# goalheart/ionic-mpnn

Measured on AMD Instinct MI355X. Metric: molecule-graph pairs/sec (fwd), batch 4096 per MI355X, higher is better.
Workload: dtype f32 (bf16x9 emulation)

## Files before the change

### include/impnn.h

```cpp
#ifndef IMPNN_H_
#define IMPNN_H_

#include <stddef.h>
#include <stdint.h>

#ifdef __cplusplus
extern "C" {
#endif

#define IMPNN_OK 0
#define IMPNN_E_BADARG (-1)
#define IMPNN_E_UNSUPPORTED (-2)
#define IMPNN_E_LAUNCH (-3)
#define IMPNN_E_WORKSPACE (-4)

typedef void* impnn_stream_t;

#define IMPNN_ABI_VERSION 3
int impnn_abi_version(void);
const char* impnn_last_error_string(void);
const char* impnn_target_arch(void);

int impnn_embed_gather(const int32_t* ids, const float* table, float* out, int64_t rows,
                       int32_t vocab, int32_t dim, impnn_stream_t stream);
// ... 97 lines not shown
int impnn_encoder_workspace_bytes(int32_t n_ions, int32_t B, int32_t N, int32_t E, int32_t D,
                                  int32_t K, int32_t S, int32_t Vb, int32_t mode, int32_t workgroups,
                                  size_t* bytes);
int impnn_encoder_fused(int32_t n_ions, const int32_t* const* atom_ids,
                        const int32_t* const* bond_ids, const int32_t* const* conn,
                        const float* atom_table, int32_t Va, const float* bond_table, int32_t Vb,
                        const float* const* weights, int32_t mode, float* const* pooled, int32_t B,
                        int32_t N, int32_t E, int32_t D, int32_t K, int32_t S, float ln_eps,
                        int32_t workgroups, void* workspace, size_t workspace_bytes,
                        impnn_stream_t stream);

size_t impnn_encoder_prepared_bytes(int32_t D, int32_t S, int32_t Vb, int32_t mode);
int impnn_encoder_prepare_weights(const float* weights, const float* bond_table, int32_t D, int32_t K,
                                  int32_t S, int32_t Vb, int32_t mode, void* prepared,
                                  size_t prepared_bytes, impnn_stream_t stream);
int impnn_encoder_fused_prepared(int32_t n_ions, const int32_t* const* atom_ids,
                                 const int32_t* const* bond_ids, const int32_t* const* conn,
                                 const float* atom_table, int32_t Va, const float* bond_table,
                                 int32_t Vb, const void* const* prepared, int32_t mode,
                                 float* const* pooled, int32_t B, int32_t N, int32_t E, int32_t D,
                                 int32_t K, int32_t S, float ln_eps, int32_t workgroups, void* workspace,
                                 size_t workspace_bytes, impnn_stream_t stream);

int64_t impnn_model_head_floats(int32_t kind, int32_t D, int32_t F, int32_t Mx);
int impnn_model_head(int32_t kind, const float* pooled_cat, const float* pooled_an,
                     const float* temperature, const float* head_weights, float* out, int32_t B,
                     int32_t D, int32_t F, int32_t Mx, impnn_stream_t stream);

int impnn_head_ion_mix(int32_t kind, int32_t ion, const float* pooled, const float* head_weights, float* mix,
                       int32_t M, int32_t D, int32_t F, int32_t Mx, impnn_stream_t stream);
// ... 232 lines not shown
```

### ionic_mpnn_amd/_lib.py

```python
from __future__ import annotations

import ctypes as C
import threading
from pathlib import Path

import torch

import os

_LIB_PATH = Path(os.environ.get("IMPNN_LIB") or Path(__file__).resolve().parent / "csrc" / "libimpnn.so")
_lock = threading.Lock()
_lib = None

i32, i64, u64, f32, vp, sz = C.c_int32, C.c_int64, C.c_uint64, C.c_float, C.c_void_p, C.c_size_t
PP = C.POINTER(vp)

_GU_FWD = [vp] * 10 + [f32, vp]
_GU_BWD = [vp] * 9 + [f32] + [vp] * 5 + [i64]
_ROWS = [vp, vp]
_DROP = [f32, u64, vp, i32]

SIGNATURES = {
    "impnn_abi_version": (C.c_int, []),
    "impnn_last_error_string": (C.c_char_p, []),
# ... 5 lines not shown
    "impnn_reduce_scatter_add": (C.c_int, [vp, vp, i32, vp, i32, i32, i32, i32, vp]),
    "impnn_bmm_fused": (C.c_int, [vp, vp, vp, vp, vp, i32, i32, i32, i32, i32, vp]),
    "impnn_gated_update": (C.c_int, _GU_FWD + [i64, i32, vp]),
    "impnn_gated_update_rows": (C.c_int, _GU_FWD + _ROWS + [i64, i32, vp]),
    "impnn_kept_rows": (C.c_int, [vp, vp, vp, vp, i32, i32, i32, i32, vp]),
    "impnn_row_index_fill": (C.c_int, [vp, vp, vp, vp, i32, i32, vp]),
    "impnn_global_sum_pool": (C.c_int, [vp, vp, vp, i32, i32, i32, vp]),
    "impnn_encoder_step_floats": (i64, [i32, i32]),
    "impnn_encoder_plan_overflow_offset": (sz, []),
    "impnn_encoder_workspace_bytes": (C.c_int, [i32] * 10 + [C.POINTER(sz)]),
    "impnn_encoder_fused": (C.c_int, [i32, C.POINTER(vp), C.POINTER(vp), C.POINTER(vp), vp, i32, vp, i32,
                                      C.POINTER(vp), i32, C.POINTER(vp), i32, i32, i32, i32, i32, i32, f32, i32, vp,
                                      sz, vp]),
    "impnn_encoder_prepared_bytes": (sz, [i32, i32, i32, i32]),
    "impnn_encoder_prepare_weights": (C.c_int, [vp, vp, i32, i32, i32, i32, i32, vp, sz, vp]),
    "impnn_encoder_fused_prepared": (C.c_int, [i32, C.POINTER(vp), C.POINTER(vp), C.POINTER(vp), vp, i32, vp, i32,
                                               C.POINTER(vp), i32, C.POINTER(vp), i32, i32, i32, i32, i32, i32, f32,
                                               i32, vp, sz, vp]),
    "impnn_encoder_plan": (C.c_int, [i32, C.POINTER(vp), C.POINTER(vp), C.POINTER(vp), i32, i32, i32, i32, i32, i32,
                                     i32, i32, i32, i32, vp, sz, vp, vp]),
    "impnn_encoder_run": (C.c_int, [i32, C.POINTER(vp), vp, i32, vp, i32, C.POINTER(vp), i32, C.POINTER(vp), i32, i32,
                                    i32, i32, i32, i32, f32, vp, vp, sz, vp]),
    "impnn_model_head_floats": (i64, [i32, i32, i32, i32]),
    "impnn_model_head": (C.c_int, [i32, vp, vp, vp, vp, vp, i32, i32, i32, i32, vp]),
    "impnn_head_ion_mix": (C.c_int, [i32, i32, vp, vp, vp, i32, i32, i32, i32, vp]),
    "impnn_head_grid": (C.c_int, [i32, vp, vp, vp, vp, vp, vp, i32, i32, i32, i32, i32, i32, vp]),
    "impnn_model_head_tensors": (C.c_int, [i32, vp, vp, vp, PP, vp, i32, i32, i32, i32, vp]),
    "impnn_model_head_bwd": (C.c_int, [i32, vp, vp, vp, PP, vp, vp, vp, PP, i32, i32, i32, i32, vp]),
    "impnn_model_head_bwd_max_floats": (i64, []),
    "impnn_model_head_loss_workspace_floats": (i64, [i32]),
# ... 166 lines not shown
```

### ionic_mpnn_amd/csrc/api.hip

```cpp
#include <cstring>
#include <vector>

#include <cstddef>

#include "common.h"
#include "encoder_layout.h"

namespace impnn {

char* error_buffer() {
  static thread_local char buf[512] = {0};
  return buf;
}

int fail(int code, const char* fmt, ...) {
  va_list ap;
  va_start(ap, fmt);
  vsnprintf(error_buffer(), 512, fmt, ap);
  va_end(ap);
  return code;
}

namespace {
struct Profiler {
// ... 421 lines not shown
                                  int32_t Vb, int32_t mode, void* prepared, size_t prepared_bytes,
                                  impnn_stream_t stream) {
  REQUIRE(D > 0 && K > 0 && S >= 0 && Vb > 0, "bad shape");
  REQUIRE(mode >= 0 && mode <= 3, "mode must be 0 (f32), 1 (f16x2), 2 (f32 typed) or 3 (f32x3 typed)");
  if (!encoder_fused_supported(mode, 1, 0, D, K, S, mode >= 2 ? Vb : 1))
    return fail(IMPNN_E_UNSUPPORTED, "encoder_prepare_weights: mode=%d D=%d K=%d Vb=%d not covered", mode, D, K, Vb);
  if (S == 0) return IMPNN_OK;
  REQUIRE(weights && prepared && (mode < 2 || bond_table), "null pointer");
  REQUIRE(aligned16(prepared), "prepared buffer must be 16B aligned");
  if (prepared_bytes < encoder_prepared_bytes(mode, D, S, Vb))
    return fail(IMPNN_E_WORKSPACE, "encoder_prepare_weights: buffer %zu < %zu bytes", prepared_bytes,
                encoder_prepared_bytes(mode, D, S, Vb));
  return launch_encoder_prepare(weights, bond_table, D, K, S, Vb, mode, prepared, as_stream(stream));
}

int impnn_encoder_fused_prepared(int32_t n_ions, const int32_t* const* atom_ids, const int32_t* const* bond_ids,
                                 const int32_t* const* conn, const float* atom_table, int32_t Va,
                                 const float* bond_table, int32_t Vb, const void* const* prepared, int32_t mode,
                                 float* const* pooled, int32_t B, int32_t N, int32_t E, int32_t D, int32_t K,
                                 int32_t S, float ln_eps, int32_t workgroups, void* workspace, size_t workspace_bytes,
                                 impnn_stream_t stream) {
  return encoder_common(__func__, n_ions, atom_ids, bond_ids, conn, atom_table, Va, bond_table, Vb, nullptr, prepared,
                        mode, pooled, B, N, E, D, K, S, ln_eps, workgroups, nullptr, nullptr, workspace,
                        workspace_bytes, stream);
}

int64_t impnn_model_head_floats(int32_t kind, int32_t D, int32_t F, int32_t Mx) {
  if (D <= 0 || F <= 0 || Mx <= 0 || (kind != 0 && kind != 1)) return -1;
  const int64_t common = 2 * ((int64_t)D * F + F) + 2 * ((int64_t)F * Mx + Mx);
  return common + (kind == 0 ? (int64_t)Mx * 3 + 3 : (int64_t)Mx * F + F + F + 1);
// ... 979 lines not shown
```

### ionic_mpnn_amd/csrc/common.h

```cpp
#pragma once

#include <hip/hip_runtime.h>

#include <cstdarg>
#include <cstdint>
#include <cstdio>

#include "../../include/impnn.h"

namespace impnn {

char* error_buffer();
int fail(int code, const char* fmt, ...);

inline hipStream_t as_stream(impnn_stream_t s) { return reinterpret_cast<hipStream_t>(s); }

inline int check_launch(const char* what) {
  hipError_t e = hipGetLastError();
  if (e != hipSuccess) return fail(IMPNN_E_LAUNCH, "%s: %s", what, hipGetErrorString(e));
  return IMPNN_OK;
}

inline bool aligned16(const void* p) { return (reinterpret_cast<uintptr_t>(p) & 15u) == 0; }

// ... 361 lines not shown
  const float* atom_table;
  const float* bond_table;
  int Va, Vb, B, N, E, D, K, S;
  float ln_eps;
  void* workspace;
  size_t workspace_bytes;
};
bool encoder_fused_supported(int mode, int N, int E, int D, int K, int S, int Vb);
int encoder_workgroups(int n_ions, int B, int requested, int N, int E, int mode);
size_t encoder_fused_workspace_bytes(int mode, int n_ions, int B, int N, int E, int D, int S, int Vb, int nwg);
int launch_encoder_fused(const EncoderArgs& a, hipStream_t s);
int launch_encoder_phase(const EncoderArgs& a, hipStream_t s, bool plan_phase);
size_t encoder_prepared_bytes(int mode, int D, int S, int Vb);
int launch_encoder_prepare(const float* weights, const float* bond_table, int D, int K, int S, int Vb, int mode,
                           void* prepared, hipStream_t s);
int ensure_lds_limit(const void* kern, int slot);
int device_compute_units();
inline int gu_wide_tile_rows(int64_t rows) { return rows < 8192 ? 16 : 64; }
bool encoder_wide_supported(int N, int E, int D, int K, int S, int Vb);
size_t encoder_wide_workspace_bytes(int n_ions, int B, int N, int E, int D, int S, int Vb, bool x3);
size_t encoder_wide_prepared_bytes(int D, int S, int Vb, bool x3);
int launch_encoder_wide_prepare(const float* weights, const float* bond_table, int D, int K, int S, int Vb, bool x3,
                                void* prepared, hipStream_t s);
int launch_encoder_wide(const EncoderArgs& a, hipStream_t s);

}
```

### ionic_mpnn_amd/csrc/encoder_fused.hip

```cpp
#include <atomic>
#include <cstdlib>

#include "encoder_device.h"
#include "encoder_layout.h"

namespace impnn {
namespace enc {

namespace {

struct H8 {
  half8 hi, lo;
};
__device__ __forceinline__ H8 split8(const float* v) {
  typedef __fp16 h2_t __attribute__((ext_vector_type(2)));
  union U {
    h2_t h;
    unsigned u;
  };
  union {
    half8 v8;
    unsigned u[4];
  } hi, lo;
#pragma unroll
// ... 396 lines not shown
    stamp[2] = t_steps;
    stamp[3] = t_pool;
    stamp[4] = (unsigned long long)(c_end - c_begin);
    stamp[7] = __builtin_amdgcn_s_memtime();
  }
}

}

}

bool encoder_typed_supported(int N, int E, int D, int S, int Vb);
size_t encoder_typed_prepared_bytes(int S, int Vb, bool x3);
int launch_encoder_typed_prepare(const float* weights, const float* bond_table, int K, int S, int Vb, bool x3,
                                 void* prepared, hipStream_t s);
int launch_encoder_typed_run(const EncoderArgs& a, const enc::Ws& w, hipStream_t s);

bool encoder_fused_supported(int mode, int N, int E, int D, int K, int S, int Vb) {
  using namespace enc;
  if ((mode == 2 || mode == 3) && D != kD) return encoder_wide_supported(N, E, D, K, S, Vb);
  if (mode == 2 || mode == 3) return K >= 1 && encoder_typed_supported(N, E, D, S, Vb);
  if (mode != 0 && mode != 1) return false;
  if (D != kD || K < 1 || K > kKMax || S < 0) return false;
  if (N < 1 || N > 0xffff || E < 0) return false;
  if (Vb < 1 || Vb > 0xffff || (int64_t)Vb * kKMax > kTbCapFloats) return false;
  const int vrmax = vr_max_of(N, E);
  if (vrmax > kRCap / 2) return false;
  return true;
}

// ... 51 lines not shown
  return (size_t)(S > 0 ? S : 1) * enc::kImgSlot * sizeof(float);
}

int launch_encoder_prepare(const float* weights, const float* bond_table, int D, int K, int S, int Vb, int mode,
                           void* prepared, hipStream_t s) {
  if (S <= 0) return IMPNN_OK;
  if (D != enc::kD) return launch_encoder_wide_prepare(weights, bond_table, D, K, S, Vb, mode == 3, prepared, s);
  if (mode >= 2) return launch_encoder_typed_prepare(weights, bond_table, K, S, Vb, mode == 3, prepared, s);
  enc::ImageParams ip{};
  ip.weights = weights;
  ip.img = static_cast<float*>(prepared);
  ip.K = K;
  ip.mode = mode == 1 ? 1 : 0;
  ip.step_floats = impnn_encoder_step_floats(D, K);
  return enc::launch_weight_image(ip, S, s);
}

int launch_encoder_fused(const EncoderArgs& a, hipStream_t s) {
  if (a.D != enc::kD) return launch_encoder_wide(a, s);
  if (a.phases & 1)
    if (int rc = launch_encoder_phase(a, s, true)) return rc;
  if (a.phases & 2)
    if (int rc = launch_encoder_phase(a, s, false)) return rc;
  return IMPNN_OK;
}

int launch_encoder_phase(const EncoderArgs& a, hipStream_t s, bool plan_phase) {
  using namespace enc;
  const bool typed = a.mode >= 2;
  const Ws w = ws_layout(a.n_ions, a.B, a.N, a.E, a.S, a.Vb, a.nwg, typed, a.mode == 3);
// ... 81 lines not shown
```

### ionic_mpnn_amd/csrc/encoder_layout.h

```cpp
#pragma once

#include "common.h"

namespace impnn {
namespace enc {

typedef float f32x4 __attribute__((ext_vector_type(4)));
typedef _Float16 half8 __attribute__((ext_vector_type(8)));

constexpr float kSW = 256.0f;
constexpr float kSX = 16.0f;
constexpr float kAcc = kSW * kSX;

constexpr int kD = 32;
constexpr int kKMax = 8;
constexpr int kRCap = 256;
constexpr int kECap = 1024;
constexpr int kHS = 36;
constexpr int kMsgRS = 36;
constexpr int kUpdRS = 68;
constexpr int kThreads = 1024;
constexpr int kWaves = kThreads / 64;
constexpr int kTbCapFloats = 2048;

// ... 58 lines not shown
constexpr int kTVecFloatOff = kTUpdBlocks * 256;
constexpr int kTUpdFloats = kTVecFloatOff + 5 * kD;
constexpr int kTUpdSlot = 2 * kThreads * 4;
constexpr int kTUpdLds = 6400;
static_assert(kTUpdFloats <= kTUpdLds && kTUpdLds <= kTUpdSlot, "typed update image");
constexpr int kXUpdHalfs = 3 * 2 * 2 * 3 * 512;
constexpr int kXVecFloatOff = kXUpdHalfs / 2;
constexpr int kXUpdFloats = kXVecFloatOff + 5 * kD;
constexpr int kXUpdSlot = 3 * kThreads * 4;
constexpr int kXUpdLds = 9472;
static_assert(kXUpdFloats <= kXUpdLds && kXUpdLds <= kXUpdSlot, "x3 update image");
constexpr int kTMatFloats = kD * kD;
inline size_t typed_prepared_floats(int S, int Vb, bool x3 = false) {
  const size_t s = S > 0 ? S : 1;
  return s * (x3 ? kXUpdSlot : kTUpdSlot) + s * (size_t)Vb * kTMatFloats + (size_t)Vb * kTMatFloats;
}

constexpr int kShareCap = kECap;
inline int plan_vmin(int n_ions, int B, int vrmax, int nwg) {
  const int64_t span = 2 * (int64_t)n_ions * B * vrmax / (nwg > 0 ? nwg : 1) + vrmax;
  const int64_t v = (span + kShareCap - 2) / (kShareCap - 1);
  return (int)(v < 1 ? 1 : (v > kRCap ? kRCap : v));
}
constexpr int kMaxHops = 128;

constexpr int kPB = 16;

struct Ws {
  size_t img_off, rows_off, vr_off, partial_off, share_off, nsub_off, desc_off, rec_off, total;
  int nwg;
// ... 96 lines not shown
};

struct TImageParams {
  const float* weights;
  const float* bond_table;
  float* prepared;
  int K, S, Vb, x3;
  int64_t step_floats;
};

struct TEncParams {
  float* pooled[2];
  const float* atom_table;
  const float* upd[2];
  const float* tmat[2];
  const int32_t* nsub;
  const int32_t* desc;
  const unsigned char* rec;
  const PlanHeader* header;
  int n_ions, B, S, Va, Vb, max_sub;
  int atab_lds;
  int upd_slot;
  int rec_lds;
  int ecap;
  float ln_eps;
  unsigned long long* stamps;
};

__device__ __forceinline__ void lds_barrier() {
  asm volatile("s_waitcnt lgkmcnt(0)\n\ts_barrier" ::: "memory");
// ... 23 lines not shown
```

### ionic_mpnn_amd/csrc/encoder_typed.hip

```cpp
#include "encoder_device.h"
#include "encoder_layout.h"

namespace impnn {
namespace enc {

namespace {

constexpr int kOffUpd = 0;
constexpr int off_h(bool x3) { return kOffUpd + (x3 ? kXUpdLds : kTUpdLds); }
constexpr int kTHSBig3 = 32;
constexpr int off_msg(bool x3, int hs = kTHS) { return off_h(x3) + kRCap * hs; }
constexpr int off_rec(bool x3, int ecap, int hs = kTHS) { return off_msg(x3, hs) + tmsg_floats(ecap); }
constexpr size_t lds_fixed_bytes(bool x3, int Vb, int ecap, int hs = kTHS) {
  return sizeof(float) * (size_t)off_rec(x3, ecap, hs) + trec_lds_bytes(Vb, ecap);
}
static_assert(lds_fixed_bytes(true, kTVbMax, kTECap) <= 160 * 1024 && lds_fixed_bytes(false, kTVbMax, kTECapBig) <= 160 * 1024 &&
                  lds_fixed_bytes(true, kTVbMax, kTECapBig, kTHSBig3) <= 160 * 1024,
              "LDS budget");

typedef __bf16 bf16x8 __attribute__((ext_vector_type(8)));
struct B3 {
  bf16x8 p0, p1, p2;
};
__device__ __forceinline__ void split_pair(float x, float y, unsigned& w0, unsigned& w1, unsigned& w2) {
// ... 43 lines not shown

template <int ABID>
__device__ __forceinline__ f32x4 mfma1(float a, float b, f32x4 c) {
  return __builtin_amdgcn_mfma_f32_4x4x1f32(a, b, c, 3, ABID, 0);
}

typedef float f32x2v __attribute__((ext_vector_type(2)));
struct Grp {
  uint4 ge;
  f32x2v aq;
};
struct Run {
  f32x4 bq[4];
  Grp first;
};

#ifndef IMPNN_T_PF
#define IMPNN_T_PF 0
#endif
#ifndef IMPNN_T_EARLY
#define IMPNN_T_EARLY 0
#endif
constexpr int kPfWhere = IMPNN_T_PF, kRunsEarly = IMPNN_T_EARLY;

template <bool STAMPS, bool X3, int HS = kTHS>
__global__ __launch_bounds__(kThreads, kThreads / 256) void encoder_typed_kernel(TEncParams p) {
  extern __shared__ __align__(16) float smem[];
  constexpr int kUpdLds = X3 ? kXUpdLds : kTUpdLds, kUpdSlot = X3 ? kXUpdSlot : kTUpdSlot;
  constexpr int kNPf = X3 ? 3 : 2;
  float* const wupd = smem + kOffUpd;
// ... 87 lines not shown
  if (p.S == 0) {
    for (int c = c_begin; c < c_end; ++c) {
      const unsigned char* rc = p.rec + (size_t)c * kTRecBytes;
      if (8 * tid < rec_lds) reinterpret_cast<uint2*>(recl)[tid] = reinterpret_cast<const uint2*>(rc)[tid];
      const int4 dsc = reinterpret_cast<const int4*>(p.desc)[c];
      lds_barrier();
      fill_h0();
      lds_barrier();
      pool(__builtin_amdgcn_readfirstlane(dsc.y), __builtin_amdgcn_readfirstlane(dsc.x),
           __builtin_amdgcn_readfirstlane(dsc.w) >> 16);
      lds_barrier();
    }
    return;
  }

  const bool rec_big = rec_lds > kTRecPart1;
  const unsigned char* rec_c = p.rec + (size_t)c_begin * kTRecBytes;
  uint2 rec_n8 = reinterpret_cast<const uint2*>(rec_c)[tid];
  uint32_t rec_n4 = rec_big ? reinterpret_cast<const uint32_t*>(rec_c + kTRecPart1)[tid] : 0u;
  int4 dsc_next = reinterpret_cast<const int4*>(p.desc)[c_begin];

  const uint32_t* const grp_x = reinterpret_cast<const uint32_t*>(r_grp);
  const int kh = lane >> 5, f = lane & 31;
  const int boff = kh * 512 + f * 4;
  const int ysh = 8 * (lane & 3), zsh = 16 * kh;
  const int acol = 16 * kh + 2 * ((lane >> 2) & 7);

  for (int c = c_begin; c < c_end; ++c) {
    const int4 dsc = dsc_next;
    const int m0 = __builtin_amdgcn_readfirstlane(dsc.x), M = __builtin_amdgcn_readfirstlane(dsc.y);
    const int rg = __builtin_amdgcn_readfirstlane(dsc.w);
    const int R = rg & 0xffff, g = rg >> 16;
    const int ntiles = (R + 15) >> 4;
    const float* upd_g = p.upd[g];
    const float* tmat_g = p.tmat[g];
    if (8 * tid < rec_lds) reinterpret_cast<uint2*>(recl)[tid] = rec_n8;
    if (rec_big && kTRecPart1 + 4 * tid < rec_lds) reinterpret_cast<uint32_t*>(recl + kTRecPart1)[tid] = rec_n4;
    {
      const int cn = (c + 1) < c_end ? (c + 1) : c;
      const unsigned char* rn = p.rec + (size_t)cn * kTRecBytes;
      rec_n8 = reinterpret_cast<const uint2*>(rn)[tid];
      if (rec_big) rec_n4 = reinterpret_cast<const uint32_t*>(rn + kTRecPart1)[tid];
      dsc_next = reinterpret_cast<const int4*>(p.desc)[cn];
    }
    lds_barrier();
    fill_h0();
    if (tid == 0) *run_ctr = 2 * kWaves;
    lds_barrier();
    if (stamp && tid == 0) {
      const unsigned long long t = __builtin_amdgcn_s_memtime();
      t_pro += t - t_mark;
      t_mark = t;
    }
    const int nrun = __builtin_amdgcn_readfirstlane(*reinterpret_cast<const uint16_t*>(recl + kTRecNrun));

    Run P, Q;
    int gP = 0, nP = 0, gQ = 0, nQ = 0;
    bool haveP = false, haveQ = false;
    const bool sP = wave < nrun, sQ = wave + kWaves < nrun;
    const int sgP = __builtin_amdgcn_readfirstlane(r_runs[sP ? wave : 0]);
    const int snP = __builtin_amdgcn_readfirstlane(r_runs[(sP ? wave : 0) + 1]) - sgP;
// ... 8 lines not shown
      for (int i = 0; i < kNPf; ++i) pf[i] = ld4(upd_g + (int64_t)s_ * kUpdSlot + 4 * (tid + i * kThreads));
    };
    auto fetch_P = [&](int s_) {
      const float* tm = tmat_g + (size_t)s_ * p.Vb * kTMatFloats;
#pragma unroll
      for (int i = 0; i < 4; ++i) P.bq[i] = ld4(tm + soP + lboffP + i * 128);
    };
    auto fetch_Q = [&](int s_) {
      const float* tm = tmat_g + (size_t)s_ * p.Vb * kTMatFloats;
#pragma unroll
      for (int i = 0; i < 4; ++i) Q.bq[i] = ld4(tm + soQ + lboffQ + i * 128);
    };
    if (kPfWhere != 0) fetch_pf(0);
    if (kRunsEarly >= 1) fetch_P(0);
    if (kRunsEarly >= 2) fetch_Q(0);
    for (int s = 0; s < p.S; ++s) {
      const float* tm_s = tmat_g + (size_t)s * p.Vb * kTMatFloats;
      __builtin_amdgcn_s_setprio(2);
      {
        const float* const abase = hbuf + acol;
        auto load_group = [&](int e, Grp& G) {
          G.ge = r_grp[e];
          const int src = __builtin_amdgcn_ubfe(G.ge.y, ysh, 8);
          G.aq = *reinterpret_cast<const f32x2v*>(abase + src * HS);
        };
        auto compute = [&](const Grp& G, const f32x4 (&bq)[4]) {
          f32x4 acc0 = {0.f, 0.f, 0.f, 0.f}, acc1 = acc0;
#ifndef IMPNN_DIAG_NO_MSG_MFMA
          acc0 = mfma1<0>(G.aq[0], bq[0][0], acc0);
          acc1 = mfma1<0>(G.aq[1], bq[0][1], acc1);
          acc0 = mfma1<1>(G.aq[0], bq[0][2], acc0);
          acc1 = mfma1<1>(G.aq[1], bq[0][3], acc1);
          acc0 = mfma1<2>(G.aq[0], bq[1][0], acc0);
          acc1 = mfma1<2>(G.aq[1], bq[1][1], acc1);
          acc0 = mfma1<3>(G.aq[0], bq[1][2], acc0);
          acc1 = mfma1<3>(G.aq[1], bq[1][3], acc1);
          acc0 = mfma1<4>(G.aq[0], bq[2][0], acc0);
          acc1 = mfma1<4>(G.aq[1], bq[2][1], acc1);
          acc0 = mfma1<5>(G.aq[0], bq[2][2], acc0);
          acc1 = mfma1<5>(G.aq[1], bq[2][3], acc1);
          acc0 = mfma1<6>(G.aq[0], bq[3][0], acc0);
          acc1 = mfma1<6>(G.aq[1], bq[3][1], acc1);
          acc0 = mfma1<7>(G.aq[0], bq[3][2], acc0);
          acc1 = mfma1<7>(G.aq[1], bq[3][3], acc1);
#else
          acc0[0] = G.aq[0] + bq[0][0] + bq[3][3];
          acc1[1] = G.aq[1] + bq[1][1] + bq[2][2];
#endif
          float x0 = acc0[0] + acc1[0], x1 = acc0[1] + acc1[1], x2 = acc0[2] + acc1[2], x3 = acc0[3] + acc1[3];
          asm volatile("s_nop 1\n\tv_permlane32_swap_b32 %0, %1\n\tv_permlane32_swap_b32 %2, %3"
                       : "+v"(x0), "+v"(x1), "+v"(x2), "+v"(x3));
          msg[__builtin_amdgcn_ubfe(G.ge.z, zsh, 16) ^ f] = x0 + x1;
          msg[__builtin_amdgcn_ubfe(G.ge.w, zsh, 16) ^ f] = x2 + x3;
        };
        auto run_type = [&](int g_, int n_, Run& Rn) {
          const int end = g_ + n_;
          Grp T;
          int e = g_;
          while (true) {
            if (e + 1 < end) load_group(e + 1, T);
            compute(Rn.first, Rn.bq);
            if (++e >= end) break;
            if (e + 1 < end) load_group(e + 1, Rn.first);
            compute(T, Rn.bq);
            if (++e >= end) break;
          }
        };
        auto fetch = [&](bool have, int r, int& g_, int& n_, Run& Rn, const float* tm) {
// ... 5 lines not shown
#pragma unroll
          for (int i = 0; i < 4; ++i) Rn.bq[i] = ld4(bp + i * 128);
        };
        auto next_run = [&]() {
          int r = 0;
          if (lane == 0) r = atomicAdd(run_ctr, 1);
          return __builtin_amdgcn_readfirstlane(r);
        };
        auto take = [&](int r, int& g_, int& n_, Run& Rn) {
          fetch(true, r, g_, n_, Rn, tm_s);
          load_group(g_, Rn.first);
        };
        auto landed = [](f32x4 (&b)[4]) {
          asm volatile("" : "+v"(b[0]), "+v"(b[1]), "+v"(b[2]), "+v"(b[3]) : : "memory");
        };
        if (kPfWhere == 0) fetch_pf(s);
        if (kRunsEarly < 1) fetch_P(s);
        if (kRunsEarly < 2) fetch_Q(s);
        haveP = sP; gP = sgP; nP = snP;
        haveQ = sQ; gQ = sgQ; nQ = snQ;
        if (haveP) load_group(gP, P.first);
        if (haveQ) load_group(gQ, Q.first);
        if (haveP) {
          if (!haveQ) {
            landed(P.bq);
            run_type(gP, nP, P);
          } else {
            while (true) {
              landed(P.bq);
              run_type(gP, nP, P);
              const int rP = next_run();
// ... 211 lines not shown
int launch_encoder_typed_prepare(const float* weights, const float* bond_table, int K, int S, int Vb, bool x3,
                                 void* prepared, hipStream_t s) {
  if (S <= 0) return IMPNN_OK;
  enc::TImageParams ip{};
  ip.weights = weights;
  ip.bond_table = bond_table;
  ip.prepared = static_cast<float*>(prepared);
  ip.K = K;
  ip.S = S;
  ip.Vb = Vb;
  ip.x3 = x3 ? 1 : 0;
  ip.step_floats = impnn_encoder_step_floats(enc::kD, K);
  return enc::launch_typed_image(ip, s);
}

int launch_encoder_typed_run(const EncoderArgs& a, const enc::Ws& w, hipStream_t s) {
  using namespace enc;
  char* base = static_cast<char*>(a.workspace);
  TEncParams ep{};
  const size_t S1 = a.S > 0 ? a.S : 1;
  const bool x3 = a.mode == 3;
  const size_t uslot = x3 ? kXUpdSlot : kTUpdSlot;
  for (int g = 0; g < a.n_ions; ++g) {
    const float* prep;
    if (a.prepared[g]) {
      if (!aligned16(a.prepared[g])) return fail(IMPNN_E_BADARG, "encoder_fused: prepared weights must be 16B aligned");
      prep = static_cast<const float*>(a.prepared[g]);
    } else {
      float* img = reinterpret_cast<float*>(base + w.img_off) + (size_t)g * typed_prepared_floats(a.S, a.Vb, x3);
      if (int rc = launch_encoder_typed_prepare(a.weights[g], a.bond_table, a.K, a.S, a.Vb, x3, img, s)) return rc;
      prep = img;
    }
    ep.upd[g] = prep;
    ep.tmat[g] = prep + S1 * uslot;
    ep.pooled[g] = a.pooled[g];
  }
  ep.atom_table = a.atom_table;
  ep.nsub = reinterpret_cast<const int32_t*>(base + w.nsub_off);
  ep.desc = reinterpret_cast<const int32_t*>(base + w.desc_off);
  ep.rec = reinterpret_cast<const unsigned char*>(base + w.rec_off);
  ep.header = reinterpret_cast<const PlanHeader*>(base);
  ep.n_ions = a.n_ions; ep.B = a.B; ep.S = a.S; ep.Va = a.Va; ep.Vb = a.Vb; ep.max_sub = w.max_sub;
  ep.ln_eps = a.ln_eps;
  ep.stamps = nullptr;
  {
    size_t sb = 0;
    void* sp = debug_stamp_buffer(&sb);
    if (sp && sb >= (size_t)w.nwg * 32 * sizeof(unsigned long long)) ep.stamps = static_cast<unsigned long long*>(sp);
  }
// ... 21 lines not shown
```

### ionic_mpnn_amd/model.py

```python
from __future__ import annotations

import os

import numpy as np
import torch

from . import data
from . import layers as L
from . import ops

INPUT_NAMES = ["cat_atom", "cat_bond", "cat_connectivity", "an_atom", "an_bond", "an_connectivity", "temperature"]


TWO_STREAM_MAX_BATCH = 4096
TRAIN_ROW_LIST_MIN_ROWS = int(os.environ.get("IMPNN_TRAIN_ROW_LIST_MIN_ROWS", 4096))


ION_KEYS = ("atom", "bond", "connectivity")
GRID_OUTPUT_BUDGET = 1 << 28
GRID_MAX_TEMPERATURES = 4096
GRID_GATHER_PAIRS = 1 << 18
SCREEN_MAX_K = ops.SELECT_MAX_K
SCREEN_MAX_PAIRS = (1 << 32) - 1

# ... 420 lines not shown
    def _packed_head(self):
        if getattr(self, "_head_packed", None) is None:
            with torch.no_grad():
                self._head_packed = torch.cat([t.reshape(-1) for t in self._head_tensors()]).contiguous()
        return self._head_packed

    def _transfer_image(self):
        if self._transfer_grid_image is None:
            with torch.no_grad():
                self._transfer_grid_image = ops.transfer_grid_prepare(self._head_tensors(), self._transfer_cfg(False))
        return self._transfer_grid_image

    def _prepared_weights(self, mode):
        if mode not in self._prepared:
            self._prepared[mode] = [ops.prepare_encoder_weights(pk, self.bond_emb.embeddings, self.atom_dim,
                                                                self.bond_dim, self.num_steps, mode)
                                    if pk is not None else None for pk in self._packed_weights()]
        return self._prepared[mode]

    def _packed_weights(self):
        if self._packed is None:
            packed = []
            for p in ("cat", "an"):
                br = self.branches[p]
                steps = []
                for i in range(self.num_steps):
                    w = br["update"][i]._weights
                    steps.append({"bond_transform": br["bmm"][i].bond_transform,
                                  "Wz": w["dense_z/kernel"], "bz": w["dense_z/bias"],
                                  "Wr": w["dense_r/kernel"], "br": w["dense_r/bias"],
                                  "Wh": w["dense_h/kernel"], "bh": w["dense_h/bias"],
# ... 720 lines not shown
```

### ionic_mpnn_amd/ops.py

```python
from __future__ import annotations

import ctypes as C

import numpy as np
import torch

from . import _lib, data
from ._lib import check, f32c, i32c, ptr, require_gpu, stream_ptr

LN_EPS = 1e-3
DEBUG_VALIDATE = False


def _wants_grad(*tensors):
    return torch.is_grad_enabled() and any(isinstance(t, torch.Tensor) and t.requires_grad for t in tensors)


class NoBackward(NotImplementedError):
    """Raised when a forward-only entry (dense bond_state message, fused encoder) is asked for gradients."""


def embed_gather(ids, table):
    if _wants_grad(table):
        from . import autograd
# ... 382 lines not shown
def split_mode_degree_limit(atom_table, bond_table, steps, D):
    if not steps:
        return float("inf")
    gmax = max(float(s["gamma"].abs().max()) for s in steps)
    bmax = max(float(s["beta"].abs().max()) for s in steps)
    wmax = max(float(s[k].abs().max()) for s in steps for k in ("bond_transform", "Wz", "Wr", "Wh"))
    l1 = max(float(s["bond_transform"].abs().sum(dim=(0, 2)).max()) for s in steps)
    hmax = float(atom_table.abs().max()) + len(steps) * ((D - 1) ** 0.5 * gmax + bmax)
    cmax = float(bond_table.abs().max())
    if wmax * SPLIT_SW >= FP16_MAX or hmax * SPLIT_SX >= FP16_MAX:
        return 0.0
    per_deg = SPLIT_SX * cmax * hmax * max(1.0, l1)
    return float("inf") if per_deg == 0.0 else 0.999 * FP16_MAX / per_deg


def prepare_encoder_weights(packed, bond_table, D, K, num_steps, mode="f32t"):
    require_gpu(packed, bond_table)
    packed, bond_table = f32c(packed), f32c(bond_table)
    S, Vb = int(num_steps), int(bond_table.shape[0])
    lib = _lib.load()
    nbytes = int(lib.impnn_encoder_prepared_bytes(D, S, Vb, ENCODER_MODES[mode]))
    out = torch.empty(max(nbytes, 16), dtype=torch.uint8, device=packed.device)
    with torch.cuda.device(packed.device):
        rc = lib.impnn_encoder_prepare_weights(ptr(packed), ptr(bond_table), D, K, S, Vb, ENCODER_MODES[mode],
                                               ptr(out), nbytes, stream_ptr())
    if rc == _lib.IMPNN_E_UNSUPPORTED:
        raise EncoderUnsupported(lib.impnn_last_error_string().decode())
    check(rc)
    return out


def encoder_fused(ions, atom_table, bond_table, packed_weights, num_steps, eps=LN_EPS, mode="f32t", prepared=None,
                  workgroups=0):
    n = len(ions)
    if n not in (1, 2):
        raise ValueError("1 or 2 ion branches")
    if mode not in ENCODER_MODES:
        raise ValueError(f"mode must be one of {sorted(ENCODER_MODES)}")
    atom_table, bond_table = f32c(atom_table), f32c(bond_table)
    require_gpu(atom_table, bond_table)
# ... 677 lines not shown
```

Measured before the change: 35.27 million.

## Precompute step-zero messages as an atom-by-bond-type table at weight-prepare time

At step 0 the hidden state equals the atom embedding, so each first-step message depends only on the (bond type, atom id) pair. A new prepare kernel computes every step-0 message product of the atom table and the first-step bond-type matrices, with an extra zero row for out-of-range ids, and stores it after the typed prepared image. A magic-stamped header records the shape. At run time the encoder checks the header and, when it matches, fills the step-0 message buffer by gathering table rows instead of running the MFMA message pass for that step. The cost is a larger prepared buffer (capped at 2 MB) and a stale table if the atom embeddings change without re-preparing.

```diff
diff --git a/include/impnn.h b/include/impnn.h
--- a/include/impnn.h
+++ b/include/impnn.h
@@ -135,6 +135,10 @@
 int impnn_encoder_prepare_weights(const float* weights, const float* bond_table, int32_t D, int32_t K,
                                   int32_t S, int32_t Vb, int32_t mode, void* prepared,
                                   size_t prepared_bytes, impnn_stream_t stream);
+size_t impnn_encoder_prepared_bytes_atoms(int32_t D, int32_t S, int32_t Va, int32_t Vb, int32_t mode);
+int impnn_encoder_prepare_weights_atoms(const float* weights, const float* bond_table, const float* atom_table,
+                                        int32_t Va, int32_t D, int32_t K, int32_t S, int32_t Vb, int32_t mode,
+                                        void* prepared, size_t prepared_bytes, impnn_stream_t stream);
 int impnn_encoder_fused_prepared(int32_t n_ions, const int32_t* const* atom_ids,
                                  const int32_t* const* bond_ids, const int32_t* const* conn,
                                  const float* atom_table, int32_t Va, const float* bond_table,
diff --git a/ionic_mpnn_amd/_lib.py b/ionic_mpnn_amd/_lib.py
--- a/ionic_mpnn_amd/_lib.py
+++ b/ionic_mpnn_amd/_lib.py
@@ -43,6 +43,8 @@
                                       sz, vp]),
     "impnn_encoder_prepared_bytes": (sz, [i32, i32, i32, i32]),
     "impnn_encoder_prepare_weights": (C.c_int, [vp, vp, i32, i32, i32, i32, i32, vp, sz, vp]),
+    "impnn_encoder_prepared_bytes_atoms": (sz, [i32, i32, i32, i32, i32]),
+    "impnn_encoder_prepare_weights_atoms": (C.c_int, [vp, vp, vp, i32, i32, i32, i32, i32, i32, vp, sz, vp]),
     "impnn_encoder_fused_prepared": (C.c_int, [i32, C.POINTER(vp), C.POINTER(vp), C.POINTER(vp), vp, i32, vp, i32,
                                                C.POINTER(vp), i32, C.POINTER(vp), i32, i32, i32, i32, i32, i32, f32,
                                                i32, vp, sz, vp]),
diff --git a/ionic_mpnn_amd/csrc/api.hip b/ionic_mpnn_amd/csrc/api.hip
--- a/ionic_mpnn_amd/csrc/api.hip
+++ b/ionic_mpnn_amd/csrc/api.hip
@@ -459,6 +459,27 @@
   return launch_encoder_prepare(weights, bond_table, D, K, S, Vb, mode, prepared, as_stream(stream));
 }
 
+size_t impnn_encoder_prepared_bytes_atoms(int32_t D, int32_t S, int32_t Va, int32_t Vb, int32_t mode) {
+  if (Va <= 0 || impnn_encoder_prepared_bytes(D, S, Vb, mode) == 0) return 0;
+  return encoder_prepared_bytes_atoms(mode, D, S, Va, Vb);
+}
+
+int impnn_encoder_prepare_weights_atoms(const float* weights, const float* bond_table, const float* atom_table,
+                                        int32_t Va, int32_t D, int32_t K, int32_t S, int32_t Vb, int32_t mode,
+                                        void* prepared, size_t prepared_bytes, impnn_stream_t stream) {
+  REQUIRE(D > 0 && K > 0 && S >= 0 && Vb > 0 && Va > 0, "bad shape");
+  REQUIRE(mode >= 0 && mode <= 3, "mode must be 0 (f32), 1 (f16x2), 2 (f32 typed) or 3 (f32x3 typed)");
+  if (!encoder_fused_supported(mode, 1, 0, D, K, S, mode >= 2 ? Vb : 1))
+    return fail(IMPNN_E_UNSUPPORTED, "encoder_prepare_weights_atoms: mode=%d D=%d K=%d Vb=%d not covered", mode, D, K, Vb);
+  if (S == 0) return IMPNN_OK;
+  REQUIRE(weights && prepared && atom_table && (mode < 2 || bond_table), "null pointer");
+  REQUIRE(aligned16(prepared) && aligned16(atom_table), "prepared buffer and atom_table must be 16B aligned");
+  if (prepared_bytes < encoder_prepared_bytes_atoms(mode, D, S, Va, Vb))
+    return fail(IMPNN_E_WORKSPACE, "encoder_prepare_weights_atoms: buffer %zu < %zu bytes", prepared_bytes,
+                encoder_prepared_bytes_atoms(mode, D, S, Va, Vb));
+  return launch_encoder_prepare_atoms(weights, bond_table, atom_table, Va, D, K, S, Vb, mode, prepared, as_stream(stream));
+}
+
 int impnn_encoder_fused_prepared(int32_t n_ions, const int32_t* const* atom_ids, const int32_t* const* bond_ids,
                                  const int32_t* const* conn, const float* atom_table, int32_t Va,
                                  const float* bond_table, int32_t Vb, const void* const* prepared, int32_t mode,
diff --git a/ionic_mpnn_amd/csrc/common.h b/ionic_mpnn_amd/csrc/common.h
--- a/ionic_mpnn_amd/csrc/common.h
+++ b/ionic_mpnn_amd/csrc/common.h
@@ -399,6 +399,9 @@
 size_t encoder_prepared_bytes(int mode, int D, int S, int Vb);
 int launch_encoder_prepare(const float* weights, const float* bond_table, int D, int K, int S, int Vb, int mode,
                            void* prepared, hipStream_t s);
+size_t encoder_prepared_bytes_atoms(int mode, int D, int S, int Va, int Vb);
+int launch_encoder_prepare_atoms(const float* weights, const float* bond_table, const float* atom_table, int Va, int D,
+                                 int K, int S, int Vb, int mode, void* prepared, hipStream_t s);
 int ensure_lds_limit(const void* kern, int slot);
 int device_compute_units();
 inline int gu_wide_tile_rows(int64_t rows) { return rows < 8192 ? 16 : 64; }
diff --git a/ionic_mpnn_amd/csrc/encoder_fused.hip b/ionic_mpnn_amd/csrc/encoder_fused.hip
--- a/ionic_mpnn_amd/csrc/encoder_fused.hip
+++ b/ionic_mpnn_amd/csrc/encoder_fused.hip
@@ -434,6 +434,9 @@
 size_t encoder_typed_prepared_bytes(int S, int Vb, bool x3);
 int launch_encoder_typed_prepare(const float* weights, const float* bond_table, int K, int S, int Vb, bool x3,
                                  void* prepared, hipStream_t s);
+size_t encoder_typed_prepared_bytes_atoms(int S, int Va, int Vb, bool x3);
+int launch_encoder_typed_prepare_atoms(const float* weights, const float* bond_table, const float* atom_table, int Va,
+                                       int K, int S, int Vb, bool x3, void* prepared, hipStream_t s);
 int launch_encoder_typed_run(const EncoderArgs& a, const enc::Ws& w, hipStream_t s);
 
 bool encoder_fused_supported(int mode, int N, int E, int D, int K, int S, int Vb) {
@@ -515,6 +518,18 @@
   ip.mode = mode == 1 ? 1 : 0;
   ip.step_floats = impnn_encoder_step_floats(D, K);
   return enc::launch_weight_image(ip, S, s);
+}
+
+size_t encoder_prepared_bytes_atoms(int mode, int D, int S, int Va, int Vb) {
+  if (D == enc::kD && mode >= 2) return encoder_typed_prepared_bytes_atoms(S, Va, Vb, mode == 3);
+  return encoder_prepared_bytes(mode, D, S, Vb);
+}
+
+int launch_encoder_prepare_atoms(const float* weights, const float* bond_table, const float* atom_table, int Va, int D,
+                                 int K, int S, int Vb, int mode, void* prepared, hipStream_t s) {
+  if (S > 0 && D == enc::kD && mode >= 2)
+    return launch_encoder_typed_prepare_atoms(weights, bond_table, atom_table, Va, K, S, Vb, mode == 3, prepared, s);
+  return launch_encoder_prepare(weights, bond_table, D, K, S, Vb, mode, prepared, s);
 }
 
 int launch_encoder_fused(const EncoderArgs& a, hipStream_t s) {
diff --git a/ionic_mpnn_amd/csrc/encoder_layout.h b/ionic_mpnn_amd/csrc/encoder_layout.h
--- a/ionic_mpnn_amd/csrc/encoder_layout.h
+++ b/ionic_mpnn_amd/csrc/encoder_layout.h
@@ -96,6 +96,17 @@
 inline size_t typed_prepared_floats(int S, int Vb, bool x3 = false) {
   const size_t s = S > 0 ? S : 1;
   return s * (x3 ? kXUpdSlot : kTUpdSlot) + s * (size_t)Vb * kTMatFloats + (size_t)Vb * kTMatFloats;
+}
+
+constexpr int32_t kM0Magic = 0x6d30746d;
+constexpr size_t kM0CapBytes = (size_t)2 << 20;
+struct M0Header {
+  int32_t magic, Va, Vb, S;
+};
+inline size_t m0_table_floats(int S, int Va, int Vb) {
+  if (S < 1 || Va < 1 || Vb < 1) return 0;
+  const size_t n = (size_t)Vb * ((size_t)Va + 1) * kD;
+  return n * sizeof(float) <= kM0CapBytes ? n : 0;
 }
 
 constexpr int kShareCap = kECap;
@@ -222,6 +233,7 @@
   const float* atom_table;
   const float* upd[2];
   const float* tmat[2];
+  const float* m0[2];
   const int32_t* nsub;
   const int32_t* desc;
   const unsigned char* rec;
diff --git a/ionic_mpnn_amd/csrc/encoder_typed.hip b/ionic_mpnn_amd/csrc/encoder_typed.hip
--- a/ionic_mpnn_amd/csrc/encoder_typed.hip
+++ b/ionic_mpnn_amd/csrc/encoder_typed.hip
@@ -81,6 +81,60 @@
   f32x4 bq[4];
   Grp first;
 };
+
+__device__ __forceinline__ void group_messages(const f32x2v aq, const f32x4 (&bq)[4], float& m01, float& m23) {
+  f32x4 acc0 = {0.f, 0.f, 0.f, 0.f}, acc1 = acc0;
+#ifndef IMPNN_DIAG_NO_MSG_MFMA
+  acc0 = mfma1<0>(aq[0], bq[0][0], acc0);
+  acc1 = mfma1<0>(aq[1], bq[0][1], acc1);
+  acc0 = mfma1<1>(aq[0], bq[0][2], acc0);
+  acc1 = mfma1<1>(aq[1], bq[0][3], acc1);
+  acc0 = mfma1<2>(aq[0], bq[1][0], acc0);
+  acc1 = mfma1<2>(aq[1], bq[1][1], acc1);
+  acc0 = mfma1<3>(aq[0], bq[1][2], acc0);
+  acc1 = mfma1<3>(aq[1], bq[1][3], acc1);
+  acc0 = mfma1<4>(aq[0], bq[2][0], acc0);
+  acc1 = mfma1<4>(aq[1], bq[2][1], acc1);
+  acc0 = mfma1<5>(aq[0], bq[2][2], acc0);
+  acc1 = mfma1<5>(aq[1], bq[2][3], acc1);
+  acc0 = mfma1<6>(aq[0], bq[3][0], acc0);
+  acc1 = mfma1<6>(aq[1], bq[3][1], acc1);
+  acc0 = mfma1<7>(aq[0], bq[3][2], acc0);
+  acc1 = mfma1<7>(aq[1], bq[3][3], acc1);
+#else
+  acc0[0] = aq[0] + bq[0][0] + bq[3][3];
+  acc1[1] = aq[1] + bq[1][1] + bq[2][2];
+#endif
+  float x0 = acc0[0] + acc1[0], x1 = acc0[1] + acc1[1], x2 = acc0[2] + acc1[2], x3 = acc0[3] + acc1[3];
+  asm volatile("s_nop 1\n\tv_permlane32_swap_b32 %0, %1\n\tv_permlane32_swap_b32 %2, %3"
+               : "+v"(x0), "+v"(x1), "+v"(x2), "+v"(x3));
+  m01 = x0 + x1;
+  m23 = x2 + x3;
+}
+
+__global__ __launch_bounds__(256) void typed_m0_kernel(const float* tmat0, const float* atom_table, float* m0,
+                                                       M0Header* hdr, int Va, int Vb, int S) {
+  const int lane = threadIdx.x & 63;
+  const int w = __builtin_amdgcn_readfirstlane(blockIdx.x * 4 + (threadIdx.x >> 6));
+  const int nga = (Va + 4) >> 2;
+  if (w < Vb * nga) {
+    const int v = w / nga, a0 = 4 * (w - v * nga);
+    const int kh = lane >> 5, f = lane & 31;
+    const int ai = a0 + (lane & 3);
+    f32x2v aq = {0.f, 0.f};
+    if (ai < Va) aq = *reinterpret_cast<const f32x2v*>(atom_table + (size_t)ai * kD + 16 * kh + 2 * ((lane >> 2) & 7));
+    const float* bp = tmat0 + (size_t)v * kTMatFloats + kh * 512 + f * 4;
+    f32x4 bq[4];
+#pragma unroll
+    for (int i = 0; i < 4; ++i) bq[i] = ld4(bp + i * 128);
+    float m01, m23;
+    group_messages(aq, bq, m01, m23);
+    float* row = m0 + (size_t)v * (Va + 1) * kD + f;
+    if (a0 + kh <= Va) row[(size_t)(a0 + kh) * kD] = m01;
+    if (a0 + 2 + kh <= Va) row[(size_t)(a0 + 2 + kh) * kD] = m23;
+  }
+  if (blockIdx.x == 0 && threadIdx.x == 0) *hdr = M0Header{kM0Magic, Va, Vb, S};
+}
 
 #ifndef IMPNN_T_PF
 #define IMPNN_T_PF 0
@@ -198,6 +252,16 @@
     return;
   }
 
+  unsigned tabmask = 0;
+  {
+    const M0Header t0 = *reinterpret_cast<const M0Header*>(p.upd[0] + kUpdLds);
+    if (t0.magic == kM0Magic && t0.Va == p.Va && t0.Vb == p.Vb && t0.S == p.S) tabmask |= 1u;
+    if (p.n_ions > 1) {
+      const M0Header t1 = *reinterpret_cast<const M0Header*>(p.upd[1] + kUpdLds);
+      if (t1.magic == kM0Magic && t1.Va == p.Va && t1.Vb == p.Vb && t1.S == p.S) tabmask |= 2u;
+    }
+  }
+
   const bool rec_big = rec_lds > kTRecPart1;
   const unsigned char* rec_c = p.rec + (size_t)c_begin * kTRecBytes;
   uint2 rec_n8 = reinterpret_cast<const uint2*>(rec_c)[tid];
@@ -218,6 +282,7 @@
     const int ntiles = (R + 15) >> 4;
     const float* upd_g = p.upd[g];
     const float* tmat_g = p.tmat[g];
+    const bool tab0 = (tabmask >> g) & 1u;
     if (8 * tid < rec_lds) reinterpret_cast<uint2*>(recl)[tid] = rec_n8;
     if (rec_big && kTRecPart1 + 4 * tid < rec_lds) reinterpret_cast<uint32_t*>(recl + kTRecPart1)[tid] = rec_n4;
     {
@@ -229,6 +294,33 @@
     }
     lds_barrier();
     fill_h0();
+    if (tab0) {
+      const int ngrp = __builtin_amdgcn_readfirstlane(*reinterpret_cast<const uint16_t*>(recl + kTRecCounts));
+      const float* const m0_g = p.m0[g];
+      int tl = tid;
+      asm volatile("" : "+v"(tl));
+      const unsigned u4 = 4 * (tl & 7);
+      const int i = (tl >> 3) & 3, g0 = tl >> 5;
+      constexpr int kGR = 8;
+      const unsigned dump = (unsigned)tmsg_key(p.ecap);
+      for (int gb = 0; gb < ngrp; gb += 32 * kGR) {
+        f32x4 mv[kGR];
+        unsigned dst[kGR];
+#pragma unroll
+        for (int j = 0; j < kGR; ++j) {
+          const int gi = gb + 32 * j + g0;
+          const uint4 ge = r_grp[gi < ngrp ? gi : ngrp - 1];
+          const bool ok = gi < ngrp && i < (int)__builtin_amdgcn_ubfe(ge.x, 8, 8);
+          const int id = r_rowatom[__builtin_amdgcn_ubfe(ge.y, 8 * i, 8)];
+          const unsigned col = (unsigned)id < (unsigned)p.Va ? (unsigned)id : (unsigned)p.Va;
+          const unsigned off = ((ge.x & 0xffu) * (unsigned)(p.Va + 1) + col) * kD + u4;
+          mv[j] = ld4(m0_g + (ok ? off : 0u));
+          dst[j] = (ok ? __builtin_amdgcn_ubfe(i < 2 ? ge.z : ge.w, 16 * (i & 1), 16) : dump) ^ u4;
+        }
+#pragma unroll
+        for (int j = 0; j < kGR; ++j) st4(msg + dst[j], mv[j]);
+      }
+    }
     if (tid == 0) *run_ctr = 2 * kWaves;
     lds_barrier();
     if (stamp && tid == 0) {
@@ -267,10 +359,13 @@
     if (kPfWhere != 0) fetch_pf(0);
     if (kRunsEarly >= 1) fetch_P(0);
     if (kRunsEarly >= 2) fetch_Q(0);
+    if (stamp && c == c_begin && tid == 0) stamp[13] = __builtin_amdgcn_s_memtime();
     for (int s = 0; s < p.S; ++s) {
       const float* tm_s = tmat_g + (size_t)s * p.Vb * kTMatFloats;
       __builtin_amdgcn_s_setprio(2);
-      {
+      const bool from_tab = tab0 && s == 0;
+      if (kPfWhere == 0) fetch_pf(s);
+      if (!from_tab) {
         const float* const abase = hbuf + acol;
         auto load_group = [&](int e, Grp& G) {
           G.ge = r_grp[e];
@@ -278,33 +373,10 @@
           G.aq = *reinterpret_cast<const f32x2v*>(abase + src * HS);
         };
         auto compute = [&](const Grp& G, const f32x4 (&bq)[4]) {
-          f32x4 acc0 = {0.f, 0.f, 0.f, 0.f}, acc1 = acc0;
-#ifndef IMPNN_DIAG_NO_MSG_MFMA
-          acc0 = mfma1<0>(G.aq[0], bq[0][0], acc0);
-          acc1 = mfma1<0>(G.aq[1], bq[0][1], acc1);
-          acc0 = mfma1<1>(G.aq[0], bq[0][2], acc0);
-          acc1 = mfma1<1>(G.aq[1], bq[0][3], acc1);
-          acc0 = mfma1<2>(G.aq[0], bq[1][0], acc0);
-          acc1 = mfma1<2>(G.aq[1], bq[1][1], acc1);
-          acc0 = mfma1<3>(G.aq[0], bq[1][2], acc0);
-          acc1 = mfma1<3>(G.aq[1], bq[1][3], acc1);
-          acc0 = mfma1<4>(G.aq[0], bq[2][0], acc0);
-          acc1 = mfma1<4>(G.aq[1], bq[2][1], acc1);
-          acc0 = mfma1<5>(G.aq[0], bq[2][2], acc0);
-          acc1 = mfma1<5>(G.aq[1], bq[2][3], acc1);
-          acc0 = mfma1<6>(G.aq[0], bq[3][0], acc0);
-          acc1 = mfma1<6>(G.aq[1], bq[3][1], acc1);
-          acc0 = mfma1<7>(G.aq[0], bq[3][2], acc0);
-          acc1 = mfma1<7>(G.aq[1], bq[3][3], acc1);
-#else
-          acc0[0] = G.aq[0] + bq[0][0] + bq[3][3];
-          acc1[1] = G.aq[1] + bq[1][1] + bq[2][2];
-#endif
-          float x0 = acc0[0] + acc1[0], x1 = acc0[1] + acc1[1], x2 = acc0[2] + acc1[2], x3 = acc0[3] + acc1[3];
-          asm volatile("s_nop 1\n\tv_permlane32_swap_b32 %0, %1\n\tv_permlane32_swap_b32 %2, %3"
-                       : "+v"(x0), "+v"(x1), "+v"(x2), "+v"(x3));
-          msg[__builtin_amdgcn_ubfe(G.ge.z, zsh, 16) ^ f] = x0 + x1;
-          msg[__builtin_amdgcn_ubfe(G.ge.w, zsh, 16) ^ f] = x2 + x3;
+          float m01, m23;
+          group_messages(G.aq, bq, m01, m23);
+          msg[__builtin_amdgcn_ubfe(G.ge.z, zsh, 16) ^ f] = m01;
+          msg[__builtin_amdgcn_ubfe(G.ge.w, zsh, 16) ^ f] = m23;
         };
         auto run_type = [&](int g_, int n_, Run& Rn) {
           const int end = g_ + n_;
@@ -340,7 +412,6 @@
         auto landed = [](f32x4 (&b)[4]) {
           asm volatile("" : "+v"(b[0]), "+v"(b[1]), "+v"(b[2]), "+v"(b[3]) : : "memory");
         };
-        if (kPfWhere == 0) fetch_pf(s);
         if (kRunsEarly < 1) fetch_P(s);
         if (kRunsEarly < 2) fetch_Q(s);
         haveP = sP; gP = sgP; nP = snP;
@@ -582,6 +653,23 @@
   return enc::launch_typed_image(ip, s);
 }
 
+size_t encoder_typed_prepared_bytes_atoms(int S, int Va, int Vb, bool x3) {
+  return (enc::typed_prepared_floats(S, Vb, x3) + enc::m0_table_floats(S, Va, Vb)) * sizeof(float);
+}
+
+int launch_encoder_typed_prepare_atoms(const float* weights, const float* bond_table, const float* atom_table, int Va,
+                                       int K, int S, int Vb, bool x3, void* prepared, hipStream_t s) {
+  using namespace enc;
+  if (int rc = launch_encoder_typed_prepare(weights, bond_table, K, S, Vb, x3, prepared, s)) return rc;
+  if (m0_table_floats(S, Va, Vb) == 0) return IMPNN_OK;
+  float* img = static_cast<float*>(prepared);
+  const size_t uslot = x3 ? kXUpdSlot : kTUpdSlot;
+  const int waves = Vb * ((Va + 4) >> 2);
+  typed_m0_kernel<<<(waves + 3) / 4, 256, 0, s>>>(img + (size_t)S * uslot, atom_table, img + typed_prepared_floats(S, Vb, x3),
+                                                  reinterpret_cast<M0Header*>(img + (x3 ? kXUpdLds : kTUpdLds)), Va, Vb, S);
+  return check_launch("typed_m0");
+}
+
 int launch_encoder_typed_run(const EncoderArgs& a, const enc::Ws& w, hipStream_t s) {
   using namespace enc;
   char* base = static_cast<char*>(a.workspace);
@@ -601,6 +689,7 @@
     }
     ep.upd[g] = prep;
     ep.tmat[g] = prep + S1 * uslot;
+    ep.m0[g] = prep + typed_prepared_floats(a.S, a.Vb, x3);
     ep.pooled[g] = a.pooled[g];
   }
   ep.atom_table = a.atom_table;
diff --git a/ionic_mpnn_amd/model.py b/ionic_mpnn_amd/model.py
--- a/ionic_mpnn_amd/model.py
+++ b/ionic_mpnn_amd/model.py
@@ -458,7 +458,8 @@
     def _prepared_weights(self, mode):
         if mode not in self._prepared:
             self._prepared[mode] = [ops.prepare_encoder_weights(pk, self.bond_emb.embeddings, self.atom_dim,
-                                                                self.bond_dim, self.num_steps, mode)
+                                                                self.bond_dim, self.num_steps, mode,
+                                                                atom_table=self.atom_emb.embeddings)
                                     if pk is not None else None for pk in self._packed_weights()]
         return self._prepared[mode]
 
diff --git a/ionic_mpnn_amd/ops.py b/ionic_mpnn_amd/ops.py
--- a/ionic_mpnn_amd/ops.py
+++ b/ionic_mpnn_amd/ops.py
@@ -420,16 +420,25 @@
     return float("inf") if per_deg == 0.0 else 0.999 * FP16_MAX / per_deg
 
 
-def prepare_encoder_weights(packed, bond_table, D, K, num_steps, mode="f32t"):
-    require_gpu(packed, bond_table)
+def prepare_encoder_weights(packed, bond_table, D, K, num_steps, mode="f32t", atom_table=None):
+    require_gpu(packed, bond_table, atom_table)
     packed, bond_table = f32c(packed), f32c(bond_table)
     S, Vb = int(num_steps), int(bond_table.shape[0])
     lib = _lib.load()
-    nbytes = int(lib.impnn_encoder_prepared_bytes(D, S, Vb, ENCODER_MODES[mode]))
+    if atom_table is None:
+        nbytes = int(lib.impnn_encoder_prepared_bytes(D, S, Vb, ENCODER_MODES[mode]))
+    else:
+        atom_table = f32c(atom_table)
+        Va = int(atom_table.shape[0])
+        nbytes = int(lib.impnn_encoder_prepared_bytes_atoms(D, S, Va, Vb, ENCODER_MODES[mode]))
     out = torch.empty(max(nbytes, 16), dtype=torch.uint8, device=packed.device)
     with torch.cuda.device(packed.device):
-        rc = lib.impnn_encoder_prepare_weights(ptr(packed), ptr(bond_table), D, K, S, Vb, ENCODER_MODES[mode],
-                                               ptr(out), nbytes, stream_ptr())
+        if atom_table is None:
+            rc = lib.impnn_encoder_prepare_weights(ptr(packed), ptr(bond_table), D, K, S, Vb, ENCODER_MODES[mode],
+                                                   ptr(out), nbytes, stream_ptr())
+        else:
+            rc = lib.impnn_encoder_prepare_weights_atoms(ptr(packed), ptr(bond_table), ptr(atom_table), Va, D, K, S, Vb,
+                                                         ENCODER_MODES[mode], ptr(out), nbytes, stream_ptr())
     if rc == _lib.IMPNN_E_UNSUPPORTED:
         raise EncoderUnsupported(lib.impnn_last_error_string().decode())
     check(rc)
```

After: 37.54 million, median of 6. +6.4%, better.
